# CVMI-Lab/HybridNeuralRendering

Hardware: AMD Instinct MI355X
Metric: rays/sec (fwd render) scene0241_01 at 1/2/4/8 GPU; PSNR delta vs ref (higher is better)
Workload: dtype f32

## Files before the change

hybridneuralrendering_amd/csrc/mlp.hip:

```cpp
#include <stdlib.h>

#include "hnr_h2.h"

namespace hnr {

constexpr int ML_PAD = 32;
constexpr int ML_SLOT = 8192 + ML_PAD;
constexpr int ML_WSTEP = 8192;
constexpr int ML_META_FLOATS = 4 * 128 + 4 + 4;
constexpr int ML_DESC = 4 * 128, ML_WMAX = 4 * 128 + 4;

struct MlpArgs {
    const float *A; int lda;
    const float *R; const int32_t *ridx; int ldr;
    const char *wimg;
    int wbase[4];
    int K0, N[4], act[4];
    float *C2; int ldc2;
    const float *loc_w; const int32_t *vs_item;
    const float *w2c, *Kmat, *campos, *campos_n;
    const float *fm; int H, W;
    const float *frame_w;
    const float *w_last, *b_last;
    const float *CF; int ldcf;
// ... 12 lines not shown
__device__ long long g_mlp_probe[24];
#define MLP_STAMP(i_) do { const long long t_ = clock64(); tm_[i_] += t_ - tp_; tp_ = t_; if ((i_) == 0) ++ntile_; } while (0)
#else
#define MLP_STAMP(i_) do { } while (0)
#endif
constexpr int mlp3_wgs_per_cu(int S0, int RT, int MODE) { return MODE == 1 ? (RT >= 4 ? 2 : 4) : RT >= 4 ? 1 : (RT == 1 || S0 <= 6) ? 4 : 2; }

#ifdef HNR_MLP_FULL_BARRIER
#define MLP_LDS_BARRIER() __syncthreads()
#else
#define MLP_LDS_BARRIER() asm volatile("s_waitcnt lgkmcnt(0)\n\ts_barrier" ::: "memory")
#endif
#ifndef HNR_MLP_LPR16
#define HNR_MLP_LPR16 1
#endif
template <int S0, int S1, int S2, int S3, int MODE, int RT = 4>
__global__ __launch_bounds__(256, mlp3_wgs_per_cu(S0, RT, MODE)) void mlp3_kernel(MlpArgs a)
{
    static_assert(MODE != 1 || RT == 4 || RT == 2, "the merge stage is built on 128- or 64-row tiles (32 / 16 samples x 4 views)");
    constexpr int SLOT = RT * 2048 + ML_PAD, ROWS = 32 * RT;
    constexpr int SMAX3 = S0 > S1 ? (S0 > S2 ? S0 : S2) : (S1 > S2 ? S1 : S2), SMAX = SMAX3 > S3 ? SMAX3 : S3;
    extern __shared__ __attribute__((aligned(16))) char lds[];
    const int tid = threadIdx.x, lane = tid & 63, wave = tid >> 6, h = lane >> 5, j = lane & 31;
    long long M = a.M_cap;
    if (a.counts) { const long long c = (long long)a.counts[a.count_index] * a.count_mult; if (c < M) M = c; }
    long long n_unit = 1;
    if (a.seg_stride > 0) {
        n_unit = a.counts ? (long long)a.counts[a.count_index] : a.M_cap / (a.count_mult > 0 ? a.count_mult : 1);
        if (n_unit > a.seg_stride) n_unit = a.seg_stride;
        if (n_unit < 1) n_unit = 1;
        if (M > n_unit * a.count_mult) M = n_unit * a.count_mult;
    }
    auto phys = [&](long long m) -> long long {
        if (a.seg_stride <= 0) return m;
        int q = 0;
        for (int v = 1; v < a.count_mult && v < 8; ++v) q += (m >= (long long)v * n_unit) ? 1 : 0;
        return (long long)q * a.seg_stride + (m - (long long)q * n_unit);
    };
    const int n_tiles = (int)((M + ROWS - 1) / ROWS);
    const int total_steps = S0 + S1 + S2 + S3;
    const float *meta = reinterpret_cast<const float *>(a.wimg + (size_t)total_steps * ML_WSTEP);
    const __amdgpu_buffer_rsrc_t wsrd = __builtin_amdgcn_make_buffer_rsrc(const_cast<char *>(a.wimg), 0, total_steps * ML_WSTEP, 0x00020000);
    float *exch = reinterpret_cast<float *>(lds + SMAX * SLOT);
    float *rowinv = exch + ROWS * 4;
    float *s_f = rowinv + ROWS;
    int *s_pix = reinterpret_cast<int *>(s_f + ROWS * 48);
    float *s_vm = reinterpret_cast<float *>(s_pix + ROWS), *s_w = s_vm + ROWS;
    float *s_wl = s_w + ROWS;
    constexpr bool RS = S1 <= 4 && S2 <= 4 && S3 == 0 && RT >= 2;
    constexpr int RTW = RS ? RT / 2 : RT;
    const int cw = RS ? (wave & 1) : wave, rt0 = RS ? (wave >> 1) * RTW : 0;
    const int col0 = 32 * cw + 16 * h;
    const unsigned woff = (unsigned)cw * 2048u + (unsigned)lane * 16u;
    const char *lds_b = lds + rt0 * 2048;
    const f32x2 slope2 = {a.slope, a.slope};

    if (MODE == 1) {
        for (int i = tid; i < 128; i += 256) s_wl[i] = i < a.N[2] ? a.w_last[i] : 0.f;
    }
    float tmax_run[3] = {0.f, 0.f, 0.f};
#ifdef HNR_MLP_PROBE
    long long tm_[20] = {0, 0, 0, 0, 0, 0, 0, 0, 0, 0, 0, 0, 0, 0, 0, 0, 0, 0, 0, 0}, tp_ = clock64(), ntile_ = 0;
#endif
    for (int tile = blockIdx.x; tile < n_tiles; tile += gridDim.x) {
        const long long row_base = (long long)tile * ROWS;
        int tid_t = tid;
        asm volatile("" : "+v"(tid_t));
        MLP_STAMP(0);
        float inv[RTW];
        if (MODE == 1) {
            if (tid < 2 * ROWS) {
                const int row_t = tid % ROWS, ls = row_t >> 2, v = row_t & 3;
                long long sidx = row_base / 4 + ls;
                if (sidx * 4 >= M) sidx = M / 4 - 1;
                const float *pw = a.loc_w + (size_t)a.vs_item[sidx] * 3;
                const float x = pw[0], y = pw[1], z = pw[2];
              if (tid < ROWS) {
                int px, py;
                const bool inval = hnr_project_pixel(x, y, z, a.w2c + 16 * v, a.Kmat, a.W, a.H, px, py);
                s_pix[tid] = ((v * a.H + py) * a.W + px) * 48;
                s_vm[tid] = inval ? 0.f : 1.f;
              } else {
                const float cx = x - a.campos[0], cy = y - a.campos[1], cz = z - a.campos[2];
                const float cn = sqrtf(cx * cx + cy * cy + cz * cz) + 1e-6f;
                const float nx = x - a.campos_n[3 * v], ny = y - a.campos_n[3 * v + 1], nz = z - a.campos_n[3 * v + 2];
                const float nn = sqrtf(nx * nx + ny * ny + nz * nz) + 1e-6f;
                s_f[row_t * 48 + 45] = hnr_div(nx, nn) - hnr_div(cx, cn); s_f[row_t * 48 + 46] = hnr_div(ny, nn) - hnr_div(cy, cn); s_f[row_t * 48 + 47] = hnr_div(nz, nn) - hnr_div(cz, cn);
              }
            }
            MLP_STAMP(13);
            __syncthreads();
            {
                constexpr int NF = ROWS * 12 / 256;
                float4 f4[NF];
#pragma unroll
                for (int it = 0; it < NF; ++it) {
                    const int idx = tid_t + 256 * it, row = idx / 12, q = idx - row * 12;
                    f4[it] = *reinterpret_cast<const float4 *>(a.fm + (size_t)s_pix[row] + 4 * q);
                }
#pragma unroll
                for (int it = 0; it < NF; ++it) {
                    const int idx = tid_t + 256 * it, row = idx / 12, q = idx - row * 12;
                    float *d = s_f + row * 48 + 4 * q;
                    if (q < 11) *reinterpret_cast<float4 *>(d) = f4[it]; else d[0] = f4[it].x;
                }
            }
            __syncthreads();
            if (wave < RT) {
                const float *src = s_f + (32 * wave + j) * 48 + 8 * h;
                float x[3][8];
                float m = 0.f;
#pragma unroll
                for (int s = 0; s < 3; ++s) {
// ... 18 lines not shown
            }
        } else
        {
            constexpr int COLS = 16 * S0, LPR = HNR_MLP_LPR16 && COLS == 288 ? 16 : (COLS > 128 ? 64 : (COLS > 64 ? 32 : 16)), RPI = 64 / LPR, NB = (COLS + 4 * LPR - 1) / (4 * LPR);
            const int lr = lane % LPR, sub = lane / LPR;
            constexpr int RW = 8 * RT;
            constexpr int ROWS_B = ((RW / RPI) * NB * 4 <= (RT < 4 ? 128 : 256)) ? RW : RW / 2;
            constexpr int BATCH = ROWS_B / RPI;
#pragma unroll 1
            for (int r0 = 0; r0 < RW; r0 += ROWS_B) {
                float4 v[BATCH][NB];
#pragma unroll
                for (int b = 0; b < BATCH; ++b) {
                    const int rl = RW * wave + r0 + b * RPI + sub;
                    long long row = row_base + rl;
                    if (row >= M) row = M - 1;
                    const float *src = a.A + (size_t)phys(row) * a.lda;
#pragma unroll
                    for (int nb = 0; nb < NB; ++nb) {
                        const int c = 4 * (nb * LPR + lr);
                        v[b][nb] = *reinterpret_cast<const float4 *>(src + (c + 4 <= a.lda ? c : 0));
                    }
                }
#pragma unroll
                for (int b = 0; b < BATCH; ++b) {
                    const int rl = RW * wave + r0 + b * RPI + sub;
                    float m = 0.f;
#pragma unroll
                    for (int nb = 0; nb < NB; ++nb) {
                        const int c = 4 * (nb * LPR + lr);
                        float *t = reinterpret_cast<float *>(&v[b][nb]);
#pragma unroll
                        for (int e = 0; e < 4; ++e) { t[e] = (c + e < a.K0) ? t[e] : 0.f; m = fmaxf(m, fabsf(t[e])); }
                    }
                    m = fmaxf(m, __builtin_amdgcn_update_dpp(m, m, 0xB1, 0xf, 0xf, false));
                    m = fmaxf(m, __builtin_amdgcn_update_dpp(m, m, 0x4E, 0xf, 0xf, false));
                    m = fmaxf(m, __builtin_amdgcn_update_dpp(m, m, 0x141, 0xf, 0xf, false));
                    m = fmaxf(m, __builtin_amdgcn_update_dpp(m, m, 0x140, 0xf, 0xf, false));
                    if (LPR >= 32) m = fmaxf(m, __builtin_amdgcn_update_dpp(m, m, 0x142, 0xa, 0xf, false));
                    if (LPR >= 64) m = fmaxf(m, __builtin_amdgcn_update_dpp(m, m, 0x143, 0xc, 0xf, false));
                    if (LPR == 64) m = __int_as_float(__builtin_amdgcn_readlane(__float_as_int(m), 63));
                    else if (LPR == 32) { const float m0 = __int_as_float(__builtin_amdgcn_readlane(__float_as_int(m), 31)), m1 = __int_as_float(__builtin_amdgcn_readlane(__float_as_int(m), 63)); m = sub ? m1 : m0; }
                    const int k = row_scale_exp(m);
                    const float sc = pow2f(k);
                    if (lr == 0) rowinv[rl] = pow2f(-k);
#pragma unroll
                    for (int nb = 0; nb < NB; ++nb) {
                        const int c = 4 * (nb * LPR + lr);
// ... 16 lines not shown
            const float dw0 = meta[ML_DESC + 0];
#pragma unroll
            for (int rt = 0; rt < RTW; ++rt) inv[rt] = __fmul_rn(rowinv[32 * (rt0 + rt) + j], dw0);
        }

        f32x16 acc[RTW][1];
        auto zero_acc = [&]() {
#pragma unroll
            for (int rt = 0; rt < RTW; ++rt)
#pragma unroll
                for (int r = 0; r < 16; ++r) acc[rt][0][r] = 0.f;
        };
        float4 ad[2][4];
        auto load_addend = [&](int rt) {
            long long row = row_base + 32 * (rt0 + rt) + j;
            if (row >= M) row = M - 1;
            const float *rrow = a.R + (size_t)(MODE == 1 ? row / 4 : (long long)a.ridx[phys(row)]) * a.ldr + col0;
#pragma unroll
            for (int q4 = 0; q4 < 4; ++q4) ad[rt & 1][q4] = *reinterpret_cast<const float4 *>(rrow + 4 * q4);
        };
        auto activate = [&](int layer, float (&amax)[RTW], auto with_addend) {
            constexpr bool ADD = decltype(with_addend)::value;
            f32x2 bias[8];
#pragma unroll
            for (int q = 0; q < 4; ++q) {
                const float4 b = *reinterpret_cast<const float4 *>(meta + layer * 128 + col0 + 4 * q);
                bias[2 * q] = f32x2{b.x, b.y}; bias[2 * q + 1] = f32x2{b.z, b.w};
            }
            const bool act = a.act[layer] != 0;
            if (ADD && MODE != 1) { load_addend(0); if (RTW > 1) load_addend(1); }
#pragma unroll
            for (int rt = 0; rt < RTW; ++rt) {
                float m = 0.f;
                const f32x2 inv2 = {inv[rt], inv[rt]};
#pragma unroll
                for (int q = 0; q < 8; ++q) {
                    f32x2 add = bias[q];
                    if (ADD) { const float4 t4 = ad[rt & 1][q >> 1]; add = add + ((q & 1) ? f32x2{t4.z, t4.w} : f32x2{t4.x, t4.y}); }
                    f32x2 v = f32x2_fma(f32x2{acc[rt][0][2 * q], acc[rt][0][2 * q + 1]}, inv2, add);
                    if (act) { const f32x2 sv = v * slope2; v.x = fmaxf(v.x, sv.x); v.y = fmaxf(v.y, sv.y); }
                    acc[rt][0][2 * q] = v.x; acc[rt][0][2 * q + 1] = v.y;
                    m = fmaxf(fmaxf(m, fabsf(v.x)), fabsf(v.y));
                }
                amax[rt] = m;
                if (ADD && rt + 2 < RTW) load_addend(rt + 2);
            }
        };
        auto publish = [&](int next_layer, bool active, float (&amax)[RTW]) {
#pragma unroll
            for (int rt = 0; rt < RTW; ++rt) {
                const float m = active ? fmaxf(amax[rt], __shfl_xor(amax[rt], 32)) : 0.f;
                if (h == 0) exch[(32 * (rt0 + rt) + j) * 4 + cw] = m;
            }
            __syncthreads();
            const float dw = meta[ML_DESC + next_layer];
// ... 13 lines not shown
                        split2h(vs.x, vs.y, ph[q], pm[q]);
                    }
                    char *dst = lds + (2 * cw + h) * SLOT + ((rt0 + rt) * 2) * 1024 + j * 16;
                    *reinterpret_cast<u32x4 *>(dst) = u32x4{ph[0], ph[1], ph[2], ph[3]};
                    *reinterpret_cast<u32x4 *>(dst + 512) = u32x4{ph[4], ph[5], ph[6], ph[7]};
                    *reinterpret_cast<u32x4 *>(dst + 1024) = u32x4{pm[0], pm[1], pm[2], pm[3]};
                    *reinterpret_cast<u32x4 *>(dst + 1024 + 512) = u32x4{pm[4], pm[5], pm[6], pm[7]};
                }
            }
            __syncthreads();
        };
        auto store = [&](float *C, int ldc) {
#pragma unroll
            for (int rt = 0; rt < RTW; ++rt) {
                const long long row = row_base + 32 * (rt0 + rt) + j;
                if (row < M) {
                    float *o = C + (size_t)phys(row) * ldc + col0;
#pragma unroll
                    for (int q = 0; q < 4; ++q) {
                        const int c = col0 + 4 * q;
                        if (c + 4 <= ldc)
                            *reinterpret_cast<float4 *>(o + 4 * q) = make_float4(acc[rt][0][4 * q], acc[rt][0][4 * q + 1], acc[rt][0][4 * q + 2], acc[rt][0][4 * q + 3]);
                    }
                }
            }
        };
        const bool act0 = 32 * cw < a.N[0], act1 = 32 * cw < a.N[1], act2 = 32 * cw < a.N[2];
        float amax[RTW];
        zero_acc();
        if (act0) {
            h2_mfma_layer<RTW, 1, S0, 0, ML_WSTEP, SLOT>(wsrd, a.wbase[0], woff, lds_b, lane, acc, []() {}, [&]() { if (MODE == 1) { load_addend(0); load_addend(1); } });
            MLP_STAMP(3);
            if (a.R) activate(0, amax, std::true_type{}); else activate(0, amax, std::false_type{});
            MLP_STAMP(4);
            if (MODE == 0 && a.T0) {
                store(a.T0, a.ldt0);
#pragma unroll
                for (int rt = 0; rt < RTW; ++rt) tmax_run[0] = fmaxf(tmax_run[0], amax[rt]);
            }
        }
        publish(1, act0, amax);
        MLP_STAMP(5);
        zero_acc();
        if (act1) {
            h2_mfma_layer<RTW, 1, S1, 0, ML_WSTEP, SLOT>(wsrd, a.wbase[1], woff, lds_b, lane, acc, []() {});
            MLP_STAMP(6);
            activate(1, amax, std::false_type{});
            if (MODE == 0 && a.T1) {
                store(a.T1, a.ldt1);
#pragma unroll
                for (int rt = 0; rt < RTW; ++rt) tmax_run[1] = fmaxf(tmax_run[1], amax[rt]);
            }
        }
        publish(2, act1, amax);
        MLP_STAMP(7);
        float cfv[6] = {0.f, 0.f, 0.f, 0.f, 0.f, 0.f};
        float4 wl4[4];
        zero_acc();
        if (act2) {
            h2_mfma_layer<RTW, 1, S2, 0, ML_WSTEP, SLOT>(wsrd, a.wbase[2], woff, lds_b, lane, acc, []() {});
            MLP_STAMP(8);
            activate(2, amax, std::false_type{});
            MLP_STAMP(9);
            if (MODE != 1) store(a.C, a.ldc);
            if (MODE == 0 && a.tmax) {
#pragma unroll
                for (int rt = 0; rt < RTW; ++rt) tmax_run[2] = fmaxf(tmax_run[2], amax[rt]);
            }
            MLP_STAMP(10);
        }
        if (MODE == 1) {
#pragma unroll
            for (int it = 0; it < (8 * RT * 45 + 255) / 256; ++it) {
                const int idx = tid_t + 256 * it, ls = idx / 45, ch = idx - ls * 45;
                const long long sidx = row_base / 4 + ls;
                cfv[it] = (idx < 8 * RT * 45 && sidx * 4 < M) ? a.CF[(size_t)sidx * a.ldcf + ch] : 0.f;
            }
#pragma unroll
            for (int q4 = 0; q4 < 4; ++q4) wl4[q4] = *reinterpret_cast<const float4 *>(s_wl + col0 + 4 * q4);
        }
        if (MODE == 1) {
#pragma unroll
            for (int rt = 0; rt < RTW; ++rt) {
                float d = 0.f;
                if (act2) {
#pragma unroll
                    for (int r = 0; r < 16; ++r) d = fmaf(acc[rt][0][r], reinterpret_cast<const float *>(wl4)[r], d);
                    d = __fadd_rn(d, __shfl_xor(d, 32));
                }
                if (h == 0) exch[(32 * (rt0 + rt) + j) * 4 + cw] = d;
            }
            MLP_LDS_BARRIER();
            MLP_STAMP(14);
            if (tid < ROWS) {
                float4 d4 = *reinterpret_cast<const float4 *>(exch + tid * 4);
                if (RS) { d4.z = 0.f; d4.w = 0.f; }
                const float d = __fadd_rn(__fadd_rn(d4.x, d4.y), __fadd_rn(d4.z, d4.w));
                float wv = hnr_div(1.f, 1.f + expf(-(d + a.b_last[0])));
                wv *= s_vm[tid];
                if (a.frame_w) wv *= a.frame_w[tid & 3];
                s_w[tid] = wv;
            }
            MLP_LDS_BARRIER();
            MLP_STAMP(15);
            {
#pragma unroll
                for (int it = 0; it < (8 * RT * 45 + 255) / 256; ++it) {
                    const int idx = tid_t + 256 * it, ls = idx / 45, ch = idx - ls * 45;
                    const long long sidx = row_base / 4 + ls;
                    if (idx < 8 * RT * 45 && sidx * 4 < M) {
                        float fsum = 0.f, wsum = 0.f;
#pragma unroll
                        for (int v = 0; v < 4; ++v) { const float wv = s_w[4 * ls + v]; fsum += s_f[(4 * ls + v) * 48 + ch] * wv; wsum += wv; }
                        float *o = a.X7 + (size_t)sidx * a.ld7;
                        __builtin_nontemporal_store(cfv[it], o + ch);
                        __builtin_nontemporal_store(hnr_div(fsum, wsum + 1e-6f), o + 45 + ch);
                    }
                }
                MLP_STAMP(17);
            }
        }
        if (S3 > 0) {
            publish(3, act2, amax);
            zero_acc();
            if (32 * wave < a.N[3]) {
                h2_mfma_layer<RTW, 1, (S3 > 0 ? S3 : 1), 0, ML_WSTEP, SLOT>(wsrd, a.wbase[3], woff, lds_b, lane, acc, []() {});
                activate(3, amax, std::false_type{});
                store(a.C2, a.ldc2);
            }
        }
        MLP_STAMP(11);
        __syncthreads();
        MLP_STAMP(12);
    }
    if (MODE == 0 && a.tmax) {
        __syncthreads();
#pragma unroll
        for (int l = 0; l < 3; ++l) {
            float m = tmax_run[l];
            for (int o = 32; o > 0; o >>= 1) m = fmaxf(m, __shfl_xor(m, o));
            if (lane == 0) exch[4 * l + wave] = m;
        }
        __syncthreads();
        if (tid < 3) { const float m = fmaxf(fmaxf(exch[4 * tid], exch[4 * tid + 1]), fmaxf(exch[4 * tid + 2], exch[4 * tid + 3])); if (m > 0.f) atomicMax(a.tmax + tid, __float_as_uint(m)); }
    }
#ifdef HNR_MLP_PROBE
    if (blockIdx.x == 0 && threadIdx.x == 0) { for (int i = 0; i < 20; ++i) g_mlp_probe[i] = tm_[i]; g_mlp_probe[20] = ntile_; }
#endif
// ... 53 lines not shown
    float *s_vm = reinterpret_cast<float *>(s_pix + 32), *s_w = s_vm + 32;
    unsigned *s_max = reinterpret_cast<unsigned *>(s_w + 32);
    float *s_dd = reinterpret_cast<float *>(s_max + 32);
    for (int i = tid; i < MW_WBYTES / 16; i += 64 * MW_WAVES) {
        const int s = i >> 8, cp = (i >> 6) & 3, ln = i & 63;
        *reinterpret_cast<u32x4 *>(lds + i * 16) = *reinterpret_cast<const u32x4 *>(a.wimg + (size_t)s * ML_WSTEP + cp * 1024 + ln * 16);
    }
    for (int i = tid; i < 3 * 64; i += 64 * MW_WAVES) s_bias[i] = meta[(i >> 6) * 128 + (i & 63)];
    for (int i = tid; i < 64; i += 64 * MW_WAVES) { s_wl[i] = a.w_last[i]; s_cam[i] = a.w2c[i]; }
    if (tid < 9) s_cam[64 + tid] = a.Kmat[tid];
    if (tid < 3) s_cam[76 + tid] = a.campos[tid];
    if (tid < 12) s_cam[80 + tid] = a.campos_n[tid];
    __syncthreads();
    const float dw0 = meta[ML_DESC + 0], dw1 = meta[ML_DESC + 1], dw2 = meta[ML_DESC + 2], b_last = a.b_last[0];
    const f32x2 slope2 = {a.slope, a.slope};
    for (int tile = blockIdx.x * MW_WAVES + wave; tile < n_tiles; tile += gridDim.x * MW_WAVES) {
        int lane = tid & 63;
        asm volatile("" : "+v"(lane));
        const int h = lane >> 5, j = lane & 31;
        const long long sbase = (long long)tile * 8;
        {
            const int ls = j >> 2, v = j & 3;
            long long sidx = sbase + ls;
            if (sidx >= n_samp) sidx = n_samp - 1;
            const float *pw = a.loc_w + (size_t)a.vs_item[sidx] * 3;
            const float x = pw[0], y = pw[1], z = pw[2];
            if (h == 0) {
                int px, py;
                const bool inval = hnr_project_pixel(x, y, z, s_cam + 16 * v, s_cam + 64, a.W, a.H, px, py);
                s_pix[j] = ((v * a.H + py) * a.W + px) * 48;
                s_vm[j] = inval ? 0.f : 1.f;
                s_max[j] = 0u;
            } else {
                const float *cp = s_cam + 76, *cnp = s_cam + 80 + 3 * v;
                const float cx = x - cp[0], cy = y - cp[1], cz = z - cp[2];
                const float cn = sqrtf(cx * cx + cy * cy + cz * cz) + 1e-6f;
                const float nx = x - cnp[0], ny = y - cnp[1], nz = z - cnp[2];
                const float nn = sqrtf(nx * nx + ny * ny + nz * nz) + 1e-6f;
                s_dd[j * 3] = hnr_div(nx, nn) - hnr_div(cx, cn); s_dd[j * 3 + 1] = hnr_div(ny, nn) - hnr_div(cy, cn); s_dd[j * 3 + 2] = hnr_div(nz, nn) - hnr_div(cz, cn);
            }
        }
        MW_WAVE_FENCE();
        float inv;
        {
            float4 f4[6];
#pragma unroll
            for (int it = 0; it < 6; ++it) {
                const int idx = lane + 64 * it, row = idx / 12, q = idx - row * 12;
                f4[it] = *reinterpret_cast<const float4 *>(a.fm + (size_t)s_pix[row] + 4 * q);
            }
#pragma unroll
            for (int it = 0; it < 6; ++it) {
                const int idx = lane + 64 * it, row = idx / 12, q = idx - row * 12;
                if (q == 11) { f4[it].y = s_dd[row * 3]; f4[it].z = s_dd[row * 3 + 1]; f4[it].w = s_dd[row * 3 + 2]; }
                const float m = fmaxf(fmaxf(fabsf(f4[it].x), fabsf(f4[it].y)), fmaxf(fabsf(f4[it].z), fabsf(f4[it].w)));
                atomicMax(s_max + row, __float_as_uint(m));
            }
            MW_WAVE_FENCE();
#pragma unroll
            for (int it = 0; it < 6; ++it) {
                const int idx = lane + 64 * it, row = idx / 12, q = idx - row * 12, c = 4 * q;
                const float sc = pow2f(row_scale_exp(__uint_as_float(s_max[row])));
                unsigned ph0, pm0, ph1, pm1;
                split2h(__fmul_rn(f4[it].x, sc), __fmul_rn(f4[it].y, sc), ph0, pm0);
                split2h(__fmul_rn(f4[it].z, sc), __fmul_rn(f4[it].w, sc), ph1, pm1);
                char *dst = wl + (c >> 4) * MW_SLOT + ((((c >> 3) & 1) * 32 + row) * 16) + (c & 7) * 2;
                *reinterpret_cast<uint2 *>(dst) = make_uint2(ph0, ph1);
                *reinterpret_cast<uint2 *>(dst + 1024) = make_uint2(pm0, pm1);
            }
            inv = __fmul_rn(pow2f(-row_scale_exp(__uint_as_float(s_max[j]))), dw0);
        }
        float4 ad[2][4];
        {
            long long sidx = sbase + (j >> 2);
            if (sidx >= n_samp) sidx = n_samp - 1;
            const float *rrow = a.R + (size_t)sidx * a.ldr + 16 * h;
#pragma unroll
            for (int c = 0; c < 2; ++c)
#pragma unroll
                for (int q4 = 0; q4 < 4; ++q4) ad[c][q4] = *reinterpret_cast<const float4 *>(rrow + 32 * c + 4 * q4);
        }
        MW_WAVE_FENCE();
        f32x16 acc[2];
        auto zero_acc = [&]() {
#pragma unroll
            for (int c = 0; c < 2; ++c)
#pragma unroll
                for (int r = 0; r < 16; ++r) acc[c][r] = 0.f;
        };
        auto activate = [&](int layer, auto with_addend) -> float {
// ... 64 lines not shown
                    d = fmaf(acc[c][4 * q4], w4.x, d); d = fmaf(acc[c][4 * q4 + 1], w4.y, d);
                    d = fmaf(acc[c][4 * q4 + 2], w4.z, d); d = fmaf(acc[c][4 * q4 + 3], w4.w, d);
                }
                d2[c] = __fadd_rn(d, __shfl_xor(d, 32));
            }
            const float d = __fadd_rn(d2[0], d2[1]);
            float wv = hnr_div(1.f, 1.f + expf(-(d + b_last)));
            wv *= s_vm[j];
            if (a.frame_w) wv *= a.frame_w[j & 3];
            if (h == 0) s_w[j] = wv;
        }
        MW_WAVE_FENCE();
        float *s_x7 = reinterpret_cast<float *>(wl);
#pragma unroll
        for (int it = 0; it < 2; ++it) {
            const int p = lane + 64 * it, ls = p / 12, q = p - ls * 12;
            long long sidx = sbase + ls;
            if (sidx >= n_samp) sidx = n_samp - 1;
            if (p < 96) {
                float4 fv[4];
#pragma unroll
                for (int v = 0; v < 4; ++v) fv[v] = *reinterpret_cast<const float4 *>(a.fm + (size_t)s_pix[4 * ls + v] + 4 * q);
                const float4 c4 = *reinterpret_cast<const float4 *>(a.CF + (size_t)sidx * a.ldcf + 4 * q);
                float fs[4] = {0.f, 0.f, 0.f, 0.f}, wsum = 0.f;
#pragma unroll
                for (int v = 0; v < 4; ++v) {
                    const float wv = s_w[4 * ls + v];
                    fs[0] += fv[v].x * wv; fs[1] += fv[v].y * wv; fs[2] += fv[v].z * wv; fs[3] += fv[v].w * wv;
                    wsum += wv;
                }
                const float den = wsum + 1e-6f;
                float *o = s_x7 + ls * 92;
                o[4 * q] = c4.x; o[45 + 4 * q] = hnr_div(fs[0], den);
                if (q < 11) {
                    o[4 * q + 1] = c4.y; o[4 * q + 2] = c4.z; o[4 * q + 3] = c4.w;
                    o[45 + 4 * q + 1] = hnr_div(fs[1], den); o[45 + 4 * q + 2] = hnr_div(fs[2], den); o[45 + 4 * q + 3] = hnr_div(fs[3], den);
                } else { o[90] = 0.f; o[91] = 0.f; }
            }
        }
        MW_WAVE_FENCE();
#pragma unroll
        for (int it = 0; it < 3; ++it) {
            const int idx = lane + 64 * it, ls = idx / 23, c4 = idx - ls * 23;
            const long long sidx = sbase + ls;
            if (idx < 8 * 23 && sidx < n_samp) {
                const f32x4m v = *reinterpret_cast<const f32x4m *>(s_x7 + ls * 92 + 4 * c4);
                __builtin_nontemporal_store(v, reinterpret_cast<f32x4m *>(a.X7 + (size_t)sidx * a.ld7 + 4 * c4));
            }
        }
        MW_WAVE_FENCE();
    }
}

struct MixArgs {
    const float *X7; int ld7;
    const char *wimg;
    const float *CF; int ldcf;
    const float *w_fin, *b_fin;
    const float *sigma; const int32_t *vs_item;
    const unsigned long long *counts; long long S_cap;
    float slope;
    float *Y; int ldy;
    float *decoded;
};
constexpr int MX_WAVES = 12;
// ... 11 lines not shown
    const float *meta = reinterpret_cast<const float *>(a.wimg + (size_t)12 * ML_WSTEP);
    float *s_bias = reinterpret_cast<float *>(lds + MX_WBYTES);
    float *s_fin = s_bias + 3 * 64;
    char *wl = lds + MX_SHARED + wave * MX_WAVE_LDS;
    unsigned *s_max = reinterpret_cast<unsigned *>(wl + 3 * MW_SLOT);
    for (int i = tid; i < MX_WBYTES / 16; i += 64 * MX_WAVES) {
        const int s = i >> 8, cp = (i >> 6) & 3, ln = i & 63;
        *reinterpret_cast<u32x4 *>(lds + i * 16) = *reinterpret_cast<const u32x4 *>(a.wimg + (size_t)s * ML_WSTEP + cp * 1024 + ln * 16);
    }
    for (int i = tid; i < 3 * 64; i += 64 * MX_WAVES) s_bias[i] = meta[(i >> 6) * 128 + (i & 63)];
    for (int i = tid; i < 3 * 128; i += 64 * MX_WAVES) s_fin[i] = a.w_fin[i];
    __syncthreads();
    const float dw0 = meta[ML_DESC + 0], dw1 = meta[ML_DESC + 1], dw2 = meta[ML_DESC + 2];
    const float bfin[3] = {a.b_fin[0], a.b_fin[1], a.b_fin[2]};
    const f32x2 slope2 = {a.slope, a.slope};
    for (int tile = blockIdx.x * MX_WAVES + wave; tile < n_tiles; tile += gridDim.x * MX_WAVES) {
        int lane = tid & 63;
        asm volatile("" : "+v"(lane));
        const int h = lane >> 5, j = lane & 31;
        const long long sbase = (long long)tile * 32;
        if (h == 0) s_max[j] = 0u;
        MW_WAVE_FENCE();
        float inv;
        float4 f4[12];
#pragma unroll
        for (int it = 0; it < 12; ++it) {
            const int idx = lane + 64 * it, row = idx / 24, q = idx - row * 24;
            long long sidx = sbase + row;
            if (sidx >= n_samp) sidx = n_samp - 1;
            if (q < 23) {
                f4[it] = *reinterpret_cast<const float4 *>(a.X7 + (size_t)sidx * a.ld7 + 4 * q);
            } else f4[it] = make_float4(0.f, 0.f, 0.f, 0.f);
        }
#pragma unroll
        for (int it = 0; it < 12; ++it) {
            const int idx = lane + 64 * it, row = idx / 24, q = idx - row * 24;
            if (q == 22) { f4[it].z = 0.f; f4[it].w = 0.f; }
            const float m = fmaxf(fmaxf(fabsf(f4[it].x), fabsf(f4[it].y)), fmaxf(fabsf(f4[it].z), fabsf(f4[it].w)));
            atomicMax(s_max + row, __float_as_uint(m));
        }
        MW_WAVE_FENCE();
        auto planes_half = [&](int half) {
#pragma unroll
            for (int it = 0; it < 12; ++it) {
                const int idx = lane + 64 * it, row = idx / 24, q = idx - row * 24, c = 4 * q - 48 * half;
                if (c >= 0 && c < 48) {
                    const float sc = pow2f(row_scale_exp(__uint_as_float(s_max[row])));
                    unsigned ph0, pm0, ph1, pm1;
                    split2h(__fmul_rn(f4[it].x, sc), __fmul_rn(f4[it].y, sc), ph0, pm0);
                    split2h(__fmul_rn(f4[it].z, sc), __fmul_rn(f4[it].w, sc), ph1, pm1);
                    char *dst = wl + (c >> 4) * MW_SLOT + ((((c >> 3) & 1) * 32 + row) * 16) + (c & 7) * 2;
                    *reinterpret_cast<uint2 *>(dst) = make_uint2(ph0, ph1);
                    *reinterpret_cast<uint2 *>(dst + 1024) = make_uint2(pm0, pm1);
                }
            }
        };
        planes_half(0);
        inv = __fmul_rn(pow2f(-row_scale_exp(__uint_as_float(s_max[j]))), dw0);
        MW_WAVE_FENCE();
        f32x16 acc[2];
        auto zero_acc = [&]() {
// ... 38 lines not shown
                    const f32x2 vs = f32x2{acc[c][2 * q], acc[c][2 * q + 1]} * sc2;
                    split2h(vs.x, vs.y, ph[q], pm[q]);
                }
                if (2 * c + h < 3) {
                    char *dst = wl + (2 * c + h) * MW_SLOT + j * 16;
                    *reinterpret_cast<u32x4 *>(dst) = u32x4{ph[0], ph[1], ph[2], ph[3]};
                    *reinterpret_cast<u32x4 *>(dst + 512) = u32x4{ph[4], ph[5], ph[6], ph[7]};
                    *reinterpret_cast<u32x4 *>(dst + 1024) = u32x4{pm[0], pm[1], pm[2], pm[3]};
                    *reinterpret_cast<u32x4 *>(dst + 1024 + 512) = u32x4{pm[4], pm[5], pm[6], pm[7]};
                }
            }
            MW_WAVE_FENCE();
        };
        const char *wp = lds + lane * 16, *bp = wl + lane * 16;
        long long srow = sbase + j;
        const bool ok = srow < n_samp;
        if (!ok) srow = n_samp - 1;
        zero_acc();
        mw_layer<3>(wp, bp, acc);
        MW_WAVE_FENCE();
        planes_half(1);
        MW_WAVE_FENCE();
        mw_layer<3>(wp + 3 * 4096, bp, acc);
        publish(dw1, activate(0, true));
        zero_acc();
        mw_layer<3>(wp + 6 * 4096, bp, acc);
        publish(dw2, activate(1, true));
        const float *cfrow = a.CF + (size_t)srow * a.ldcf;
        float4 cfa[2][4], cfb[8];
#pragma unroll
        for (int c = 0; c < 2; ++c)
// ... 52 lines not shown
            const float hi = vh + uh;
            rj[o] = lo + hi;
        }
        if (ok && h == 0) {
            float4 out;
            out.x = a.sigma[srow];
#pragma unroll
            for (int o = 0; o < 3; ++o) {
                const float sg = hnr_div(1.f, 1.f + expf(-(rj[o] + bfin[o])));
                const float cch = sg * (1.f + 2.f * 0.001f) - 0.001f;
                if (o == 0) out.y = cch; else if (o == 1) out.z = cch; else out.w = cch;
            }
            reinterpret_cast<float4 *>(a.decoded)[a.vs_item[srow]] = out;
        }
        MW_WAVE_FENCE();
    }
}

struct MlpPackArgs {
    const float *W[4]; int ldw[4], N[4], K[4], S[4], base[4];
    const float *b[4];
    char *out; int total_steps;
};

__global__ void mlp_wmax_kernel(MlpPackArgs a)
{
    const int l = blockIdx.y;
    unsigned *wmax = reinterpret_cast<unsigned *>(a.out + (size_t)a.total_steps * ML_WSTEP) + ML_WMAX;
    float m = 0.f;
    for (int i = blockIdx.x * blockDim.x + threadIdx.x; i < a.N[l] * a.K[l]; i += gridDim.x * blockDim.x) {
// ... 143 lines not shown
    a.C = d_C; a.ldc = ldc; a.C2 = d_C2; a.ldc2 = ldc2;
    a.T0 = d_T0; a.ldt0 = ldt0; a.T1 = d_T1; a.ldt1 = ldt1; a.tmax = d_tmax;
    a.loc_w = nullptr; a.vs_item = nullptr; a.w2c = a.Kmat = a.campos = a.campos_n = a.fm = a.frame_w = a.w_last = a.b_last = a.CF = nullptr;
    a.H = a.W = a.ldcf = a.ld7 = 0; a.X7 = nullptr;
    const int n_cu = device_num_cus();
    hipStream_t st = (hipStream_t)stream;
#define HNR_MLP3_CASE(S0_, S1_, S2_, S3_, RT_)                                                                                         \
    if (S[0] == S0_ && S[1] == S1_ && S[2] == S2_ && S[3] == S3_) {                                                                     \
        if (S1_ <= 4 && S2_ <= 4 && S3_ == 0 && RT_ >= 2 && N[2] > 64) {    \
            set_error("hnr_mlp3_forward: N[2] = %d > 64 with 64-wide hidden layers is not built", N[2]); return HNR_ERR_BADARG; }             \
        constexpr int smax3 = S0_ > S1_ ? (S0_ > S2_ ? S0_ : S2_) : (S1_ > S2_ ? S1_ : S2_), smax = smax3 > S3_ ? smax3 : S3_;          \
        constexpr int ldsb = smax * (RT_ * 2048 + ML_PAD) + 32 * RT_ * 4 * 4 + 32 * RT_ * 4;                                                       \
        const int64_t tiles = (M_cap + 32 * RT_ - 1) / (32 * RT_);                                                                      \
        const int wgs = mlp3_wgs_per_cu(S0_, RT_, 0) * n_cu, grid = (int)(tiles < wgs ? tiles : wgs);                                              \
        static PerDeviceOnce attr;                                                                                                      \
        if (attr.first()) HNR_HIP_CHECK(hipFuncSetAttribute(reinterpret_cast<const void *>(mlp3_kernel<S0_, S1_, S2_, S3_, 0, RT_>), hipFuncAttributeMaxDynamicSharedMemorySize, ldsb)); \
        mlp3_kernel<S0_, S1_, S2_, S3_, 0, RT_><<<grid, 256, ldsb, st>>>(a);                                                             \
        mlp3_probe_print(st, n_layers, K[0]);                                                                                          \
        HNR_LAUNCH_CHECK();                                                                                                             \
        return HNR_OK;                                                                                                                  \
    }
    HNR_MLP3_CASE(18, 8, 8, 0, 2)
    HNR_MLP3_CASE(18, 8, 8, 8, 2)
    HNR_MLP3_CASE(3, 4, 4, 0, 4)
    HNR_MLP3_CASE(6, 3, 3, 0, 2)
#undef HNR_MLP3_CASE
    set_error("hnr_mlp3_forward: no kernel for k steps (%d, %d, %d, %d); built: (18,8,8,0) (18,8,8,8) (3,4,4,0) (6,3,3,0)", S[0], S[1], S[2], S[3]);
    return HNR_ERR_BADARG;
}


extern "C" int hnr_merge_stage(const float *d_sample_loc_w, const int32_t *d_vs_item, const int64_t *d_counts, const float *d_w2c, const float *d_intrinsic,
// ... 79 lines not shown
```

Measured before the change: 7.935 million.

## Specialize MLP kernels for full tiles and segment mode, read args from kernarg

Splits the tile loops of the mlp3, merge-wave and decode kernels into a full-tile path with no bounds clamps and a single tail tile. Adds a compile-time SEG template flag in place of the runtime seg_stride check, reads kernel arguments through the kernarg segment pointer so they stay scalar, and turns the activation branch into a branchless slope multiply. It also hoists per-lane index divisions out of the feature-gather loops. The intent is fewer VALU instructions, branches and register use per tile, at the cost of code size and two instantiations of each kernel.

```diff
diff --git a/hybridneuralrendering_amd/csrc/mlp.hip b/hybridneuralrendering_amd/csrc/mlp.hip
--- a/hybridneuralrendering_amd/csrc/mlp.hip
+++ b/hybridneuralrendering_amd/csrc/mlp.hip
@@ -50,25 +50,26 @@
 #ifndef HNR_MLP_LPR16
 #define HNR_MLP_LPR16 1
 #endif
-template <int S0, int S1, int S2, int S3, int MODE, int RT = 4>
+template <int S0, int S1, int S2, int S3, int MODE, int RT = 4, bool SEG = false>
 __global__ __launch_bounds__(256, mlp3_wgs_per_cu(S0, RT, MODE)) void mlp3_kernel(MlpArgs a)
 {
     static_assert(MODE != 1 || RT == 4 || RT == 2, "the merge stage is built on 128- or 64-row tiles (32 / 16 samples x 4 views)");
     constexpr int SLOT = RT * 2048 + ML_PAD, ROWS = 32 * RT;
     constexpr int SMAX3 = S0 > S1 ? (S0 > S2 ? S0 : S2) : (S1 > S2 ? S1 : S2), SMAX = SMAX3 > S3 ? SMAX3 : S3;
     extern __shared__ __attribute__((aligned(16))) char lds[];
-    const int tid = threadIdx.x, lane = tid & 63, wave = tid >> 6, h = lane >> 5, j = lane & 31;
+    const int tid = threadIdx.x, lane = tid & 63, wave = __builtin_amdgcn_readfirstlane(tid >> 6), h = lane >> 5, j = lane & 31;
+    const __attribute__((address_space(4))) MlpArgs *ap = (const __attribute__((address_space(4))) MlpArgs *)__builtin_amdgcn_kernarg_segment_ptr();
     long long M = a.M_cap;
     if (a.counts) { const long long c = (long long)a.counts[a.count_index] * a.count_mult; if (c < M) M = c; }
     long long n_unit = 1;
-    if (a.seg_stride > 0) {
+    if (SEG) {
         n_unit = a.counts ? (long long)a.counts[a.count_index] : a.M_cap / (a.count_mult > 0 ? a.count_mult : 1);
         if (n_unit > a.seg_stride) n_unit = a.seg_stride;
         if (n_unit < 1) n_unit = 1;
         if (M > n_unit * a.count_mult) M = n_unit * a.count_mult;
     }
     auto phys = [&](long long m) -> long long {
-        if (a.seg_stride <= 0) return m;
+        if (!SEG) return m;
         int q = 0;
         for (int v = 1; v < a.count_mult && v < 8; ++v) q += (m >= (long long)v * n_unit) ? 1 : 0;
         return (long long)q * a.seg_stride + (m - (long long)q * n_unit);
@@ -89,7 +90,6 @@
     const int col0 = 32 * cw + 16 * h;
     const unsigned woff = (unsigned)cw * 2048u + (unsigned)lane * 16u;
     const char *lds_b = lds + rt0 * 2048;
-    const f32x2 slope2 = {a.slope, a.slope};
 
     if (MODE == 1) {
         for (int i = tid; i < 128; i += 256) s_wl[i] = i < a.N[2] ? a.w_last[i] : 0.f;
@@ -98,7 +98,11 @@
 #ifdef HNR_MLP_PROBE
     long long tm_[20] = {0, 0, 0, 0, 0, 0, 0, 0, 0, 0, 0, 0, 0, 0, 0, 0, 0, 0, 0, 0}, tp_ = clock64(), ntile_ = 0;
 #endif
-    for (int tile = blockIdx.x; tile < n_tiles; tile += gridDim.x) {
+    auto run_tile = [&](const int tile, auto full_tag) {
+        constexpr bool FULL = decltype(full_tag)::value;
+        auto ap_t = ap;
+        asm volatile("" : "+s"(ap_t));
+        const auto &ta = *ap_t;
         const long long row_base = (long long)tile * ROWS;
         int tid_t = tid;
         asm volatile("" : "+v"(tid_t));
@@ -108,18 +112,18 @@
             if (tid < 2 * ROWS) {
                 const int row_t = tid % ROWS, ls = row_t >> 2, v = row_t & 3;
                 long long sidx = row_base / 4 + ls;
-                if (sidx * 4 >= M) sidx = M / 4 - 1;
-                const float *pw = a.loc_w + (size_t)a.vs_item[sidx] * 3;
+                if (!FULL && sidx * 4 >= M) sidx = M / 4 - 1;
+                const float *pw = ta.loc_w + (size_t)ta.vs_item[sidx] * 3;
                 const float x = pw[0], y = pw[1], z = pw[2];
               if (tid < ROWS) {
                 int px, py;
-                const bool inval = hnr_project_pixel(x, y, z, a.w2c + 16 * v, a.Kmat, a.W, a.H, px, py);
-                s_pix[tid] = ((v * a.H + py) * a.W + px) * 48;
+                const bool inval = hnr_project_pixel(x, y, z, ta.w2c + 16 * v, ta.Kmat, ta.W, ta.H, px, py);
+                s_pix[tid] = ((v * ta.H + py) * ta.W + px) * 48;
                 s_vm[tid] = inval ? 0.f : 1.f;
               } else {
-                const float cx = x - a.campos[0], cy = y - a.campos[1], cz = z - a.campos[2];
+                const float cx = x - ta.campos[0], cy = y - ta.campos[1], cz = z - ta.campos[2];
                 const float cn = sqrtf(cx * cx + cy * cy + cz * cz) + 1e-6f;
-                const float nx = x - a.campos_n[3 * v], ny = y - a.campos_n[3 * v + 1], nz = z - a.campos_n[3 * v + 2];
+                const float nx = x - ta.campos_n[3 * v], ny = y - ta.campos_n[3 * v + 1], nz = z - ta.campos_n[3 * v + 2];
                 const float nn = sqrtf(nx * nx + ny * ny + nz * nz) + 1e-6f;
                 s_f[row_t * 48 + 45] = hnr_div(nx, nn) - hnr_div(cx, cn); s_f[row_t * 48 + 46] = hnr_div(ny, nn) - hnr_div(cy, cn); s_f[row_t * 48 + 47] = hnr_div(nz, nn) - hnr_div(cz, cn);
               }
@@ -132,7 +136,7 @@
 #pragma unroll
                 for (int it = 0; it < NF; ++it) {
                     const int idx = tid_t + 256 * it, row = idx / 12, q = idx - row * 12;
-                    f4[it] = *reinterpret_cast<const float4 *>(a.fm + (size_t)s_pix[row] + 4 * q);
+                    f4[it] = *reinterpret_cast<const float4 *>(ta.fm + (size_t)s_pix[row] + 4 * q);
                 }
 #pragma unroll
                 for (int it = 0; it < NF; ++it) {
@@ -181,12 +185,13 @@
                 for (int b = 0; b < BATCH; ++b) {
                     const int rl = RW * wave + r0 + b * RPI + sub;
                     long long row = row_base + rl;
-                    if (row >= M) row = M - 1;
+                    if (!FULL && row >= M) row = M - 1;
                     const float *src = a.A + (size_t)phys(row) * a.lda;
 #pragma unroll
                     for (int nb = 0; nb < NB; ++nb) {
                         const int c = 4 * (nb * LPR + lr);
-                        v[b][nb] = *reinterpret_cast<const float4 *>(src + (c + 4 <= a.lda ? c : 0));
+                        const bool kin = 4 * (nb + 1) * LPR <= 16 * (S0 - 1);
+                        v[b][nb] = *reinterpret_cast<const float4 *>(src + (kin || c + 4 <= a.lda ? c : 0));
                     }
                 }
 #pragma unroll
@@ -197,8 +202,9 @@
                     for (int nb = 0; nb < NB; ++nb) {
                         const int c = 4 * (nb * LPR + lr);
                         float *t = reinterpret_cast<float *>(&v[b][nb]);
-#pragma unroll
-                        for (int e = 0; e < 4; ++e) { t[e] = (c + e < a.K0) ? t[e] : 0.f; m = fmaxf(m, fabsf(t[e])); }
+                        const bool kin = 4 * (nb + 1) * LPR <= 16 * (S0 - 1);
+#pragma unroll
+                        for (int e = 0; e < 4; ++e) { if (!kin) t[e] = (c + e < a.K0) ? t[e] : 0.f; m = fmaxf(m, fabsf(t[e])); }
                     }
                     m = fmaxf(m, __builtin_amdgcn_update_dpp(m, m, 0xB1, 0xf, 0xf, false));
                     m = fmaxf(m, __builtin_amdgcn_update_dpp(m, m, 0x4E, 0xf, 0xf, false));
@@ -245,8 +251,8 @@
         float4 ad[2][4];
         auto load_addend = [&](int rt) {
             long long row = row_base + 32 * (rt0 + rt) + j;
-            if (row >= M) row = M - 1;
-            const float *rrow = a.R + (size_t)(MODE == 1 ? row / 4 : (long long)a.ridx[phys(row)]) * a.ldr + col0;
+            if (!FULL && row >= M) row = M - 1;
+            const float *rrow = ta.R + (size_t)(MODE == 1 ? row / 4 : (long long)ta.ridx[phys(row)]) * ta.ldr + col0;
 #pragma unroll
             for (int q4 = 0; q4 < 4; ++q4) ad[rt & 1][q4] = *reinterpret_cast<const float4 *>(rrow + 4 * q4);
         };
@@ -258,7 +264,8 @@
                 const float4 b = *reinterpret_cast<const float4 *>(meta + layer * 128 + col0 + 4 * q);
                 bias[2 * q] = f32x2{b.x, b.y}; bias[2 * q + 1] = f32x2{b.z, b.w};
             }
-            const bool act = a.act[layer] != 0;
+            const float sl = ta.act[layer] != 0 ? a.slope : 1.f;
+            const f32x2 sl2 = {sl, sl};
             if (ADD && MODE != 1) { load_addend(0); if (RTW > 1) load_addend(1); }
 #pragma unroll
             for (int rt = 0; rt < RTW; ++rt) {
@@ -269,7 +276,8 @@
                     f32x2 add = bias[q];
                     if (ADD) { const float4 t4 = ad[rt & 1][q >> 1]; add = add + ((q & 1) ? f32x2{t4.z, t4.w} : f32x2{t4.x, t4.y}); }
                     f32x2 v = f32x2_fma(f32x2{acc[rt][0][2 * q], acc[rt][0][2 * q + 1]}, inv2, add);
-                    if (act) { const f32x2 sv = v * slope2; v.x = fmaxf(v.x, sv.x); v.y = fmaxf(v.y, sv.y); }
+                    const f32x2 sv = v * sl2;
+                    v.x = fmaxf(v.x, sv.x); v.y = fmaxf(v.y, sv.y);
                     acc[rt][0][2 * q] = v.x; acc[rt][0][2 * q + 1] = v.y;
                     m = fmaxf(fmaxf(m, fabsf(v.x)), fabsf(v.y));
                 }
@@ -313,27 +321,33 @@
 #pragma unroll
             for (int rt = 0; rt < RTW; ++rt) {
                 const long long row = row_base + 32 * (rt0 + rt) + j;
-                if (row < M) {
+                if (FULL || row < M) {
                     float *o = C + (size_t)phys(row) * ldc + col0;
-#pragma unroll
-                    for (int q = 0; q < 4; ++q) {
-                        const int c = col0 + 4 * q;
-                        if (c + 4 <= ldc)
+                    if (32 * cw + 32 <= ldc) {
+#pragma unroll
+                        for (int q = 0; q < 4; ++q)
                             *reinterpret_cast<float4 *>(o + 4 * q) = make_float4(acc[rt][0][4 * q], acc[rt][0][4 * q + 1], acc[rt][0][4 * q + 2], acc[rt][0][4 * q + 3]);
+                    } else {
+                        const int c0 = 32 * cw + 16 * ((tid_t >> 5) & 1);
+#pragma unroll
+                        for (int q = 0; q < 4; ++q) {
+                            if (c0 + 4 * q + 4 <= ldc)
+                                *reinterpret_cast<float4 *>(o + 4 * q) = make_float4(acc[rt][0][4 * q], acc[rt][0][4 * q + 1], acc[rt][0][4 * q + 2], acc[rt][0][4 * q + 3]);
+                        }
                     }
                 }
             }
         };
-        const bool act0 = 32 * cw < a.N[0], act1 = 32 * cw < a.N[1], act2 = 32 * cw < a.N[2];
+        const bool act0 = 32 * cw < ta.N[0], act1 = 32 * cw < ta.N[1], act2 = 32 * cw < ta.N[2];
         float amax[RTW];
         zero_acc();
         if (act0) {
-            h2_mfma_layer<RTW, 1, S0, 0, ML_WSTEP, SLOT>(wsrd, a.wbase[0], woff, lds_b, lane, acc, []() {}, [&]() { if (MODE == 1) { load_addend(0); load_addend(1); } });
+            h2_mfma_layer<RTW, 1, S0, 0, ML_WSTEP, SLOT>(wsrd, ta.wbase[0], woff, lds_b, lane, acc, []() {}, [&]() { if (MODE == 1) { load_addend(0); load_addend(1); } });
             MLP_STAMP(3);
-            if (a.R) activate(0, amax, std::true_type{}); else activate(0, amax, std::false_type{});
+            if (ta.R) activate(0, amax, std::true_type{}); else activate(0, amax, std::false_type{});
             MLP_STAMP(4);
-            if (MODE == 0 && a.T0) {
-                store(a.T0, a.ldt0);
+            if (MODE == 0 && ta.T0) {
+                store(ta.T0, ta.ldt0);
 #pragma unroll
                 for (int rt = 0; rt < RTW; ++rt) tmax_run[0] = fmaxf(tmax_run[0], amax[rt]);
             }
@@ -342,11 +356,11 @@
         MLP_STAMP(5);
         zero_acc();
         if (act1) {
-            h2_mfma_layer<RTW, 1, S1, 0, ML_WSTEP, SLOT>(wsrd, a.wbase[1], woff, lds_b, lane, acc, []() {});
+            h2_mfma_layer<RTW, 1, S1, 0, ML_WSTEP, SLOT>(wsrd, ta.wbase[1], woff, lds_b, lane, acc, []() {});
             MLP_STAMP(6);
             activate(1, amax, std::false_type{});
-            if (MODE == 0 && a.T1) {
-                store(a.T1, a.ldt1);
+            if (MODE == 0 && ta.T1) {
+                store(ta.T1, ta.ldt1);
 #pragma unroll
                 for (int rt = 0; rt < RTW; ++rt) tmax_run[1] = fmaxf(tmax_run[1], amax[rt]);
             }
@@ -357,12 +371,12 @@
         float4 wl4[4];
         zero_acc();
         if (act2) {
-            h2_mfma_layer<RTW, 1, S2, 0, ML_WSTEP, SLOT>(wsrd, a.wbase[2], woff, lds_b, lane, acc, []() {});
+            h2_mfma_layer<RTW, 1, S2, 0, ML_WSTEP, SLOT>(wsrd, ta.wbase[2], woff, lds_b, lane, acc, []() {});
             MLP_STAMP(8);
             activate(2, amax, std::false_type{});
             MLP_STAMP(9);
-            if (MODE != 1) store(a.C, a.ldc);
-            if (MODE == 0 && a.tmax) {
+            if (MODE != 1) store(ta.C, ta.ldc);
+            if (MODE == 0 && ta.tmax) {
 #pragma unroll
                 for (int rt = 0; rt < RTW; ++rt) tmax_run[2] = fmaxf(tmax_run[2], amax[rt]);
             }
@@ -373,7 +387,7 @@
             for (int it = 0; it < (8 * RT * 45 + 255) / 256; ++it) {
                 const int idx = tid_t + 256 * it, ls = idx / 45, ch = idx - ls * 45;
                 const long long sidx = row_base / 4 + ls;
-                cfv[it] = (idx < 8 * RT * 45 && sidx * 4 < M) ? a.CF[(size_t)sidx * a.ldcf + ch] : 0.f;
+                cfv[it] = (idx < 8 * RT * 45 && (FULL || sidx * 4 < M)) ? ta.CF[(size_t)sidx * ta.ldcf + ch] : 0.f;
             }
 #pragma unroll
             for (int q4 = 0; q4 < 4; ++q4) wl4[q4] = *reinterpret_cast<const float4 *>(s_wl + col0 + 4 * q4);
@@ -395,9 +409,9 @@
                 float4 d4 = *reinterpret_cast<const float4 *>(exch + tid * 4);
                 if (RS) { d4.z = 0.f; d4.w = 0.f; }
                 const float d = __fadd_rn(__fadd_rn(d4.x, d4.y), __fadd_rn(d4.z, d4.w));
-                float wv = hnr_div(1.f, 1.f + expf(-(d + a.b_last[0])));
+                float wv = hnr_div(1.f, 1.f + expf(-(d + ta.b_last[0])));
                 wv *= s_vm[tid];
-                if (a.frame_w) wv *= a.frame_w[tid & 3];
+                if (ta.frame_w) wv *= ta.frame_w[tid & 3];
                 s_w[tid] = wv;
             }
             MLP_LDS_BARRIER();
@@ -407,11 +421,11 @@
                 for (int it = 0; it < (8 * RT * 45 + 255) / 256; ++it) {
                     const int idx = tid_t + 256 * it, ls = idx / 45, ch = idx - ls * 45;
                     const long long sidx = row_base / 4 + ls;
-                    if (idx < 8 * RT * 45 && sidx * 4 < M) {
+                    if (idx < 8 * RT * 45 && (FULL || sidx * 4 < M)) {
                         float fsum = 0.f, wsum = 0.f;
 #pragma unroll
                         for (int v = 0; v < 4; ++v) { const float wv = s_w[4 * ls + v]; fsum += s_f[(4 * ls + v) * 48 + ch] * wv; wsum += wv; }
-                        float *o = a.X7 + (size_t)sidx * a.ld7;
+                        float *o = ta.X7 + (size_t)sidx * ta.ld7;
                         __builtin_nontemporal_store(cfv[it], o + ch);
                         __builtin_nontemporal_store(hnr_div(fsum, wsum + 1e-6f), o + 45 + ch);
                     }
@@ -422,15 +436,21 @@
         if (S3 > 0) {
             publish(3, act2, amax);
             zero_acc();
-            if (32 * wave < a.N[3]) {
-                h2_mfma_layer<RTW, 1, (S3 > 0 ? S3 : 1), 0, ML_WSTEP, SLOT>(wsrd, a.wbase[3], woff, lds_b, lane, acc, []() {});
+            if (32 * wave < ta.N[3]) {
+                h2_mfma_layer<RTW, 1, (S3 > 0 ? S3 : 1), 0, ML_WSTEP, SLOT>(wsrd, ta.wbase[3], woff, lds_b, lane, acc, []() {});
                 activate(3, amax, std::false_type{});
-                store(a.C2, a.ldc2);
+                store(ta.C2, ta.ldc2);
             }
         }
         MLP_STAMP(11);
         __syncthreads();
         MLP_STAMP(12);
+    };
+    {
+        const int n_full = (int)(M / ROWS);
+        int tile = blockIdx.x;
+        for (; tile < n_full; tile += gridDim.x) run_tile(tile, std::true_type{});
+        if (tile < n_tiles) run_tile(tile, std::false_type{});
     }
     if (MODE == 0 && a.tmax) {
         __syncthreads();
@@ -514,7 +534,8 @@
     __syncthreads();
     const float dw0 = meta[ML_DESC + 0], dw1 = meta[ML_DESC + 1], dw2 = meta[ML_DESC + 2], b_last = a.b_last[0];
     const f32x2 slope2 = {a.slope, a.slope};
-    for (int tile = blockIdx.x * MW_WAVES + wave; tile < n_tiles; tile += gridDim.x * MW_WAVES) {
+    auto run_tile = [&](const int tile, auto full_tag) {
+        constexpr bool FULL = decltype(full_tag)::value;
         int lane = tid & 63;
         asm volatile("" : "+v"(lane));
         const int h = lane >> 5, j = lane & 31;
@@ -522,7 +543,7 @@
         {
             const int ls = j >> 2, v = j & 3;
             long long sidx = sbase + ls;
-            if (sidx >= n_samp) sidx = n_samp - 1;
+            if (!FULL && sidx >= n_samp) sidx = n_samp - 1;
             const float *pw = a.loc_w + (size_t)a.vs_item[sidx] * 3;
             const float x = pw[0], y = pw[1], z = pw[2];
             if (h == 0) {
@@ -541,17 +562,20 @@
             }
         }
         MW_WAVE_FENCE();
+        int r3[3], q3[3];
+#pragma unroll
+        for (int k = 0; k < 3; ++k) { const int idx = lane + 64 * k; r3[k] = idx / 12; q3[k] = idx - r3[k] * 12; }
         float inv;
         {
             float4 f4[6];
 #pragma unroll
             for (int it = 0; it < 6; ++it) {
-                const int idx = lane + 64 * it, row = idx / 12, q = idx - row * 12;
+                const int row = r3[it % 3] + 16 * (it / 3), q = q3[it % 3];
                 f4[it] = *reinterpret_cast<const float4 *>(a.fm + (size_t)s_pix[row] + 4 * q);
             }
 #pragma unroll
             for (int it = 0; it < 6; ++it) {
-                const int idx = lane + 64 * it, row = idx / 12, q = idx - row * 12;
+                const int row = r3[it % 3] + 16 * (it / 3), q = q3[it % 3];
                 if (q == 11) { f4[it].y = s_dd[row * 3]; f4[it].z = s_dd[row * 3 + 1]; f4[it].w = s_dd[row * 3 + 2]; }
                 const float m = fmaxf(fmaxf(fabsf(f4[it].x), fabsf(f4[it].y)), fmaxf(fabsf(f4[it].z), fabsf(f4[it].w)));
                 atomicMax(s_max + row, __float_as_uint(m));
@@ -559,7 +583,7 @@
             MW_WAVE_FENCE();
 #pragma unroll
             for (int it = 0; it < 6; ++it) {
-                const int idx = lane + 64 * it, row = idx / 12, q = idx - row * 12, c = 4 * q;
+                const int row = r3[it % 3] + 16 * (it / 3), q = q3[it % 3], c = 4 * q;
                 const float sc = pow2f(row_scale_exp(__uint_as_float(s_max[row])));
                 unsigned ph0, pm0, ph1, pm1;
                 split2h(__fmul_rn(f4[it].x, sc), __fmul_rn(f4[it].y, sc), ph0, pm0);
@@ -573,7 +597,7 @@
         float4 ad[2][4];
         {
             long long sidx = sbase + (j >> 2);
-            if (sidx >= n_samp) sidx = n_samp - 1;
+            if (!FULL && sidx >= n_samp) sidx = n_samp - 1;
             const float *rrow = a.R + (size_t)sidx * a.ldr + 16 * h;
 #pragma unroll
             for (int c = 0; c < 2; ++c)
@@ -668,9 +692,9 @@
         float *s_x7 = reinterpret_cast<float *>(wl);
 #pragma unroll
         for (int it = 0; it < 2; ++it) {
-            const int p = lane + 64 * it, ls = p / 12, q = p - ls * 12;
+            const int p = lane + 64 * it, ls = r3[it], q = q3[it];
             long long sidx = sbase + ls;
-            if (sidx >= n_samp) sidx = n_samp - 1;
+            if (!FULL && sidx >= n_samp) sidx = n_samp - 1;
             if (p < 96) {
                 float4 fv[4];
 #pragma unroll
@@ -697,12 +721,18 @@
         for (int it = 0; it < 3; ++it) {
             const int idx = lane + 64 * it, ls = idx / 23, c4 = idx - ls * 23;
             const long long sidx = sbase + ls;
-            if (idx < 8 * 23 && sidx < n_samp) {
+            if (idx < 8 * 23 && (FULL || sidx < n_samp)) {
                 const f32x4m v = *reinterpret_cast<const f32x4m *>(s_x7 + ls * 92 + 4 * c4);
                 __builtin_nontemporal_store(v, reinterpret_cast<f32x4m *>(a.X7 + (size_t)sidx * a.ld7 + 4 * c4));
             }
         }
         MW_WAVE_FENCE();
+    };
+    {
+        const int n_full = (int)(n_samp / 8);
+        int tile = blockIdx.x * MW_WAVES + wave;
+        for (; tile < n_full; tile += gridDim.x * MW_WAVES) run_tile(tile, std::true_type{});
+        if (tile < n_tiles) run_tile(tile, std::false_type{});
     }
 }
 
@@ -744,37 +774,48 @@
     const float dw0 = meta[ML_DESC + 0], dw1 = meta[ML_DESC + 1], dw2 = meta[ML_DESC + 2];
     const float bfin[3] = {a.b_fin[0], a.b_fin[1], a.b_fin[2]};
     const f32x2 slope2 = {a.slope, a.slope};
-    for (int tile = blockIdx.x * MX_WAVES + wave; tile < n_tiles; tile += gridDim.x * MX_WAVES) {
+    auto run_tile = [&](const int tile, auto full_tag) {
+        constexpr bool FULL = decltype(full_tag)::value;
         int lane = tid & 63;
         asm volatile("" : "+v"(lane));
         const int h = lane >> 5, j = lane & 31;
         const long long sbase = (long long)tile * 32;
         if (h == 0) s_max[j] = 0u;
         MW_WAVE_FENCE();
+        int r3[3], q3[3];
+#pragma unroll
+        for (int k = 0; k < 3; ++k) { const int idx = lane + 64 * k; r3[k] = idx / 12; q3[k] = idx - r3[k] * 12; }
+        const float *xrow[3];
+#pragma unroll
+        for (int k = 0; k < 3; ++k) xrow[k] = a.X7 + (size_t)(sbase + r3[k]) * a.ld7 + 4 * q3[k];
         float inv;
         float4 f4[12];
 #pragma unroll
         for (int it = 0; it < 12; ++it) {
-            const int idx = lane + 64 * it, row = idx / 24, q = idx - row * 24;
-            long long sidx = sbase + row;
-            if (sidx >= n_samp) sidx = n_samp - 1;
-            if (q < 23) {
-                f4[it] = *reinterpret_cast<const float4 *>(a.X7 + (size_t)sidx * a.ld7 + 4 * q);
+            const int hf = it / 6, radd = 16 * ((it / 3) & 1), row = r3[it % 3] + radd, q = q3[it % 3] + 12 * hf;
+            const float *src = xrow[it % 3] + (size_t)radd * a.ld7 + 48 * hf;
+            if (!FULL) {
+                long long sidx = sbase + row;
+                if (sidx >= n_samp) sidx = n_samp - 1;
+                src = a.X7 + (size_t)sidx * a.ld7 + 4 * q;
+            }
+            if (hf == 0 || q < 23) {
+                f4[it] = *reinterpret_cast<const float4 *>(src);
             } else f4[it] = make_float4(0.f, 0.f, 0.f, 0.f);
         }
 #pragma unroll
         for (int it = 0; it < 12; ++it) {
-            const int idx = lane + 64 * it, row = idx / 24, q = idx - row * 24;
-            if (q == 22) { f4[it].z = 0.f; f4[it].w = 0.f; }
+            const int hf = it / 6, row = r3[it % 3] + 16 * ((it / 3) & 1), q = q3[it % 3] + 12 * hf;
+            if (hf == 1 && q == 22) { f4[it].z = 0.f; f4[it].w = 0.f; }
             const float m = fmaxf(fmaxf(fabsf(f4[it].x), fabsf(f4[it].y)), fmaxf(fabsf(f4[it].z), fabsf(f4[it].w)));
             atomicMax(s_max + row, __float_as_uint(m));
         }
         MW_WAVE_FENCE();
         auto planes_half = [&](int half) {
 #pragma unroll
-            for (int it = 0; it < 12; ++it) {
-                const int idx = lane + 64 * it, row = idx / 24, q = idx - row * 24, c = 4 * q - 48 * half;
-                if (c >= 0 && c < 48) {
+            for (int i6 = 0; i6 < 6; ++i6) {
+                const int it = 6 * half + i6, row = r3[it % 3] + 16 * ((it / 3) & 1), c = 4 * q3[it % 3];
+                {
                     const float sc = pow2f(row_scale_exp(__uint_as_float(s_max[row])));
                     unsigned ph0, pm0, ph1, pm1;
                     split2h(__fmul_rn(f4[it].x, sc), __fmul_rn(f4[it].y, sc), ph0, pm0);
@@ -843,7 +884,7 @@
         };
         const char *wp = lds + lane * 16, *bp = wl + lane * 16;
         long long srow = sbase + j;
-        const bool ok = srow < n_samp;
+        const bool ok = FULL || srow < n_samp;
         if (!ok) srow = n_samp - 1;
         zero_acc();
         mw_layer<3>(wp, bp, acc);
@@ -926,6 +967,12 @@
             reinterpret_cast<float4 *>(a.decoded)[a.vs_item[srow]] = out;
         }
         MW_WAVE_FENCE();
+    };
+    {
+        const int n_full = (int)(n_samp / 32);
+        int tile = blockIdx.x * MX_WAVES + wave;
+        for (; tile < n_full; tile += gridDim.x * MX_WAVES) run_tile(tile, std::true_type{});
+        if (tile < n_tiles) run_tile(tile, std::false_type{});
     }
 }
 
@@ -1099,8 +1146,12 @@
         const int64_t tiles = (M_cap + 32 * RT_ - 1) / (32 * RT_);                                                                      \
         const int wgs = mlp3_wgs_per_cu(S0_, RT_, 0) * n_cu, grid = (int)(tiles < wgs ? tiles : wgs);                                              \
         static PerDeviceOnce attr;                                                                                                      \
-        if (attr.first()) HNR_HIP_CHECK(hipFuncSetAttribute(reinterpret_cast<const void *>(mlp3_kernel<S0_, S1_, S2_, S3_, 0, RT_>), hipFuncAttributeMaxDynamicSharedMemorySize, ldsb)); \
-        mlp3_kernel<S0_, S1_, S2_, S3_, 0, RT_><<<grid, 256, ldsb, st>>>(a);                                                             \
+        if (attr.first()) {                                                                                                             \
+            HNR_HIP_CHECK(hipFuncSetAttribute(reinterpret_cast<const void *>(mlp3_kernel<S0_, S1_, S2_, S3_, 0, RT_, false>), hipFuncAttributeMaxDynamicSharedMemorySize, ldsb)); \
+            HNR_HIP_CHECK(hipFuncSetAttribute(reinterpret_cast<const void *>(mlp3_kernel<S0_, S1_, S2_, S3_, 0, RT_, true>), hipFuncAttributeMaxDynamicSharedMemorySize, ldsb)); \
+        }                                                                                                                               \
+        if (seg_stride > 0) mlp3_kernel<S0_, S1_, S2_, S3_, 0, RT_, true><<<grid, 256, ldsb, st>>>(a);                                  \
+        else mlp3_kernel<S0_, S1_, S2_, S3_, 0, RT_, false><<<grid, 256, ldsb, st>>>(a);                                                \
         mlp3_probe_print(st, n_layers, K[0]);                                                                                          \
         HNR_LAUNCH_CHECK();                                                                                                             \
         return HNR_OK;                                                                                                                  \
```

Measured after the change: 8.012 million, median of 6. About the same (+1.0%).
